# visanalexandru/felics

Hardware: AMD Instinct MI355X
Metric: encode MPix/s on 4K 8-bit grayscale batch (bit-exact); % HBM-read roofline (higher is better)
Workload: dtype u8

## Files before the change

felics_amd/csrc/felics_api.cpp:

```cpp
#include <hip/hip_runtime.h>

#include <chrono>
#include <cstdio>
#include <cstdlib>
#include <cstring>
#include <thread>
#include <type_traits>
#include <string>
#include <algorithm>
#include <new>
#include <tuple>
#include <vector>

#include "../../include/felics.h"
#include "felics_kernels.h"

using namespace felics;

namespace {

enum Stage { ST_PLANES = 0, ST_HIST, ST_OFFSETS, ST_SCATTER, ST_SPINE, ST_ASSIGN, ST_LENGTHS, ST_BITSCAN, ST_ZERO, ST_PACK,
             ST_WIDE_KEYS, ST_WIDE_SORT, ST_WIDE_CHAINS, ST_COUNT };
const char *kStageNames[ST_COUNT] = {"planes", "hist", "offsets", "scatter", "spine", "assign", "lengths", "bitscan", "zero", "pack",
                                     "wide_keys", "wide_sort", "wide_chains"};
static_assert(ST_COUNT <= FELICS_MAX_STAGES, "felics.h promises at most FELICS_MAX_STAGES stages");

constexpr int SLICES = 12;
constexpr uint64_t PASS_MAX_CHAINS = 1u << 23;
constexpr int EV_PAIRS = SLICES + 2;
constexpr int MAX_LANES = 4;
constexpr int DEFAULT_LANES = 2;
int lanes_from_env() {
    if (const char *e = getenv("FELICS_LANES")) return std::max(1, std::min(atoi(e), MAX_LANES));
    return DEFAULT_LANES;
}

struct DevBuf {
    void *p = nullptr;
    size_t cap = 0;
};

struct Lane {
    hipStream_t stream = nullptr;
    hipStream_t front = nullptr;
    hipStream_t kstream = nullptr;
    hipStream_t tail = nullptr;
    hipEvent_t slice_done[SLICES] = {};
    hipEvent_t spine_done[SLICES] = {};
    hipEvent_t assign_done[SLICES] = {};
    hipEvent_t ev[ST_COUNT][EV_PAIRS][2] = {};
    int ev_used[ST_COUNT] = {};
    hipEvent_t sized = nullptr;
    hipEvent_t span_begin = nullptr, span_end = nullptr;
    uint64_t *h_sizes = nullptr;
    size_t h_sizes_cap = 0;
    DevBuf planes, counts, chain_prog, scalars, evs, pix_of, k_map, k_sorted, block_state, group_bits, tile_slots, desc,
        tile_bits, tile_bitoff, plane_sums, image_bytes, image_off, partial, status, edge_first, edge_last, pscratch;
    DevBuf wrecs[2], wtile_cnt, wmeta, whist, wdigtot, heads, wlong;
    uint32_t epoch = 0;
    bool pending = false;
    bool finished = false;
    size_t p_n = 0;
    const void *p_pixels = nullptr;
    uint32_t p_w = 0, p_h = 0;
    int p_color = 0, p_depth = 0;
    uint8_t *p_out = nullptr;
    size_t p_cap = 0;
    uint64_t p_slot = 0;
    std::vector<uint64_t> r_off, r_len;
    int r_rc = 0;
    int nslices = SLICES;
    bool m_tickets = false;
    bool m_fused = false;
    bool queued = false;
    Geometry g;
    size_t first_image = 0;
    const void *d_planes = nullptr;
    DevBuf mtable;
    PlaneGeom *h_table = nullptr;
    size_t h_table_cap = 0;
};

}

struct felics_ctx {
    int device = -1;
    int next_lane = 0;
    int nlanes = DEFAULT_LANES;
    int slices_blocking = 3;
    int slices_queued = 2;
    bool pack_tickets = false;
    bool two_pass = false;
    bool own_tails = false;
    bool serial = false;
    bool test_timeout = false;
    bool test_lookback = false;
    bool scatter_ballot = false;
    bool cap_max = false;
    bool test_tile_cap = false;
    bool test_scatter_order = false;
    bool poison = false;
    bool trace = false;
    int timeout_s = 120;
    bool failed = false;
    felics_stats stats = {};
    Lane lanes[MAX_LANES];
    std::string err;
    bool profiling = false;
    float stage_ms[ST_COUNT] = {};
    float span_ms = 0.f;
    int stage_launches[ST_COUNT] = {};
    DevBuf in, out;
    hipStream_t copy_in = nullptr, copy_out = nullptr;
    std::vector<hipEvent_t> h2d_done;
    hipEvent_t wait_before_submit = nullptr;
    DevBuf mix_in, mix_stage, mix_out, mix_redo;
    DevBuf own;
    DevBuf dec_meta, dec_planes;
    DevBuf dec_planes16;
    DevBuf dec_lane_table;
    DevBuf dec_table;
    uint32_t dec_epoch = 0;
};

namespace {

int hip_fail(felics_ctx *ctx, hipError_t e, const char *what) {
    char buf[256];
    snprintf(buf, sizeof buf, "%s: %s", what, hipGetErrorString(e));
    if (ctx) ctx->err = buf;
    return FELICS_E_HIP;
}

#define HIP_TRY(ctx, call)                                          \
    do {                                                            \
        hipError_t e__ = (call);                                    \
        if (e__ != hipSuccess) return hip_fail(ctx, e__, #call);    \
    } while (0)

int wait_event(felics_ctx *ctx, hipEvent_t ev, const char *what) {
    const auto t0 = std::chrono::steady_clock::now();
    if (ctx->test_timeout) {
        ctx->err = std::string(what) + ": timed out waiting for the GPU; the context is unusable from here on";
        ctx->failed = true;
        ctx->stats.failed = 1;
        return FELICS_E_HIP;
    }
    for (uint32_t spins = 0;; spins++) {
        const hipError_t e = hipEventQuery(ev);
        if (e == hipSuccess) return FELICS_OK;
        if (e != hipErrorNotReady) return hip_fail(ctx, e, what);
        if (spins > 2000) std::this_thread::sleep_for(std::chrono::microseconds(50));
        if ((spins & 1023) == 1023 &&
            std::chrono::steady_clock::now() - t0 > std::chrono::seconds(ctx->timeout_s)) {
            ctx->err = std::string(what) + ": timed out waiting for the GPU; the context is unusable from here on";
            ctx->failed = true;
            ctx->stats.failed = 1;
            return FELICS_E_HIP;
        }
    }
}

int sync_lane(felics_ctx *ctx, Lane &l) {
    if (l.front) HIP_TRY(ctx, hipStreamSynchronize(l.front));
    if (l.stream) HIP_TRY(ctx, hipStreamSynchronize(l.stream));
    if (l.kstream) HIP_TRY(ctx, hipStreamSynchronize(l.kstream));
    if (l.tail) HIP_TRY(ctx, hipStreamSynchronize(l.tail));
    return FELICS_OK;
}

int reserve(felics_ctx *ctx, DevBuf &b, size_t bytes) {
    if (bytes <= b.cap) return FELICS_OK;
    if (b.p) {
        HIP_TRY(ctx, hipFree(b.p));
        b.p = nullptr;
        b.cap = 0;
// ... 7 lines not shown
int reserve_zeroed(felics_ctx *ctx, DevBuf &b, size_t bytes) {
    if (bytes <= b.cap) return FELICS_OK;
    int rc = reserve(ctx, b, bytes);
    if (rc) return rc;
    HIP_TRY(ctx, hipMemset(b.p, 0, b.cap));
    return FELICS_OK;
}

void release(DevBuf &b) {
    if (b.p) (void)hipFree(b.p);
    b.p = nullptr;
    b.cap = 0;
}

struct StageTimer {
    felics_ctx *ctx;
    Lane &lane;
    int st;
    hipStream_t stream;
    int slot = -1;
    bool exact;
    StageTimer(felics_ctx *c, Lane &l, int s, hipStream_t on, bool single_kernel = false)
        : ctx(c), lane(l), st(s), stream(on), exact(single_kernel) {
        if (ctx->profiling && lane.ev_used[st] < EV_PAIRS) {
            slot = lane.ev_used[st]++;
            if (exact)
                g_launch_timing = LaunchTiming{lane.ev[st][slot][0], lane.ev[st][slot][1]};
            else
                (void)hipEventRecord(lane.ev[st][slot][0], stream);
        }
    }
    ~StageTimer() {
        if (slot >= 0) {
            if (!exact) {
                (void)hipEventRecord(lane.ev[st][slot][1], stream);
            } else if (g_launch_timing.start) {
                g_launch_timing = LaunchTiming{};
                lane.ev_used[st]--;
            }
        }
        if (ctx->trace) {
            hipError_t e = hipStreamSynchronize(stream);
            fprintf(stderr, "[felics] %s done (%s)\n", kStageNames[st], hipGetErrorString(e));
        }
    }
};

int check_args(uint32_t w, uint32_t h, int color, int depth) {
    if (color != FELICS_COLOR_GRAY && color != FELICS_COLOR_RGB) return FELICS_E_INVALID_COLOR_TYPE;
    if (depth != FELICS_DEPTH_8 && depth != FELICS_DEPTH_16) return FELICS_E_INVALID_PIXEL_DEPTH;
    if ((uint64_t)w * h > 0xFFFFFFFFull) return FELICS_E_INVALID_DIMENSIONS;
    return FELICS_OK;
}

void header_bytes(uint8_t *o, uint32_t w, uint32_t h, int color, int depth) {
    memcpy(o, "FLCS", 4);
    o[4] = (uint8_t)color;
    o[5] = (uint8_t)depth;
    for (int i = 0; i < 4; i++) {
        o[6 + i] = (uint8_t)(w >> (24 - 8 * i));
        o[10 + i] = (uint8_t)(h >> (24 - 8 * i));
    }
}

template <typename T, typename ET>
int run_lane(felics_ctx *ctx, Lane &l, uint8_t *d_out, uint64_t slot_stride) {
    const Geometry &g = l.g;
    const int ns = l.nslices;
    const size_t nsamples = (size_t)g.nplanes * g.npix;
    int rc = 0;
    const bool fused = (slot_stride != 0 || g.mixed != nullptr) && !ctx->two_pass;
    const uint32_t cap = ctx->cap_max ? tile_cap_max(g.nctx, g.npix) : ctx->test_tile_cap ? std::min(4u * REC, tile_cap_max(g.nctx, g.npix)) : tile_cap_default(g.nctx, g.npix);
    const size_t ptiles = (size_t)g.nplanes * g.sort_tiles;
    const size_t slots = ptiles * cap, recs = slots / REC;
    const size_t nchains = (size_t)g.nplanes * g.nctx;
    if ((rc = reserve(ctx, l.evs, slots * sizeof(ET) + STAGE_PAD)) != 0) return rc;
    if ((rc = reserve(ctx, l.pix_of, slots * 2 + STAGE_PAD)) != 0) return rc;
    if ((rc = reserve(ctx, l.k_sorted, slots + STAGE_PAD)) != 0) return rc;
    if ((rc = reserve(ctx, l.counts, ptiles * g.nctx * 4)) != 0) return rc;
    if ((rc = reserve(ctx, l.tile_slots, ptiles * 4)) != 0) return rc;
    if ((rc = reserve(ctx, l.desc, recs * 8 + 64)) != 0) return rc;
    if ((rc = reserve(ctx, l.block_state, recs * 16 + 64)) != 0) return rc;
    if ((rc = reserve(ctx, l.partial, (size_t)SLICES * nchains * 8)) != 0) return rc;
    if ((rc = reserve(ctx, l.chain_prog, nchains * 32)) != 0) return rc;
    if ((rc = reserve(ctx, l.scalars, 64 + 4 * (SLICES + 2) + 4 * SLICES)) != 0) return rc;
    if (!fused && (rc = reserve(ctx, l.k_map, nsamples + STAGE_PAD)) != 0) return rc;
    if (!fused && (rc = reserve(ctx, l.group_bits, (size_t)g.nplanes * g.pack_tiles * PACK_THREADS * 2)) != 0) return rc;
    if ((rc = reserve(ctx, l.tile_bits, (size_t)g.nplanes * g.pack_tiles * 4)) != 0) return rc;
    if ((rc = reserve(ctx, l.tile_bitoff, (size_t)g.nplanes * g.pack_tiles * 8)) != 0) return rc;
    if ((rc = reserve(ctx, l.plane_sums, (size_t)g.nplanes * 16)) != 0) return rc;
    if ((rc = reserve(ctx, l.image_bytes, (size_t)g.nimages * 8)) != 0) return rc;
    if ((rc = reserve(ctx, l.image_off, (size_t)(g.nimages + 1) * 8)) != 0) return rc;
    if ((rc = reserve_zeroed(ctx, l.status, (size_t)g.nplanes * g.pack_tiles * 8)) != 0) return rc;
    if ((rc = reserve(ctx, l.edge_first, (size_t)g.nplanes * g.pack_tiles * 4)) != 0) return rc;
    if ((rc = reserve(ctx, l.edge_last, (size_t)g.nplanes * g.pack_tiles * 4)) != 0) return rc;
    const size_t hs = (size_t)g.nimages * 2 + 1;
    if (hs > l.h_sizes_cap) {
        if (l.h_sizes) HIP_TRY(ctx, hipHostFree(l.h_sizes));
        l.h_sizes = nullptr;
        HIP_TRY(ctx, hipHostMalloc((void **)&l.h_sizes, hs * 8 + 64, hipHostMallocDefault));
        l.h_sizes_cap = hs;
    }
    hipStream_t s = l.stream, f = l.front, ks = l.kstream, tl = l.tail;
    if (ctx->serial) f = ks = tl = s;
    const T *d_planes = (const T *)l.d_planes;
    auto *chain_state = (uint32_t *)l.chain_prog.p;
    auto *plane_carry = (uint64_t *)l.plane_sums.p;
    auto *plane_base = plane_carry + g.nplanes;
    if (++l.epoch >= 0x03FFFFFFu) l.epoch = 1;
    if ((l.epoch & 0x3FFFFu) == 0) HIP_TRY(ctx, hipMemsetAsync(l.status.p, 0, l.status.cap, f));
    const uint32_t epoch = l.epoch;
    PackTarget target{d_out, slot_stride, nullptr, 0};
    if (fused && g.planes_per_image > 1) {
        target.plane_slot = ((uint64_t)g.npix + g.npix / 4 + 64 + 15) & ~15ull;
        if ((rc = reserve(ctx, l.pscratch, (size_t)(target.plane_slot * g.nimages * (g.planes_per_image - 1)))) != 0) return rc;
        target.scratch = (uint8_t *)l.pscratch.p;
    }
    uint32_t *d_error = (uint32_t *)l.scalars.p + 8;
    uint32_t *d_flags = (uint32_t *)l.scalars.p + 9;
    uint32_t *d_tickets = (uint32_t *)l.scalars.p + 16;
    uint32_t *d_nrec = (uint32_t *)l.scalars.p + 16 + SLICES + 2;
    const TileLocal<ET> tloc{(ET *)l.evs.p, (uint16_t *)l.pix_of.p, (uint8_t *)l.k_sorted.p, (uint32_t *)l.counts.p, (uint32_t *)l.tile_slots.p, cap};
    l.m_tickets = ctx->pack_tickets;
    l.m_fused = fused;

    uint32_t bounds[SLICES + 1];
    for (int q = 0; q <= ns; q++) bounds[q] = (uint32_t)((uint64_t)g.sort_tiles * q / ns);
    auto slice_of = [&](int q) {
        const size_t r0 = (size_t)bounds[q] * g.nplanes * (cap / REC);
        return ChainSlice{(uint2 *)l.desc.p + r0, (uint2 *)l.partial.p + (size_t)q * nchains, d_nrec + q, (uint4 *)l.block_state.p};
    };
    if (ctx->poison) {
        DevBuf *bufs[] = {&l.evs, &l.pix_of, &l.k_sorted, &l.counts, &l.tile_slots, &l.desc, &l.block_state, &l.partial, &l.k_map,
                          &l.group_bits, &l.tile_bits, &l.tile_bitoff, &l.edge_first, &l.edge_last, &l.pscratch};
        for (DevBuf *b : bufs)
            if (b->p) HIP_TRY(ctx, hipMemsetAsync(b->p, 0xA5, b->cap, f));
    }
    HIP_TRY(ctx, hipMemsetAsync(chain_state, 0, nchains * 32, f));
    HIP_TRY(ctx, hipMemsetAsync(d_flags, 0, 4, f));
    HIP_TRY(ctx, hipMemsetAsync(d_nrec, 0, 4 * SLICES, f));
    const uint32_t front_mode = ctx->scatter_ballot ? FRONT_SAFE_RANK : ctx->test_scatter_order ? FRONT_TEST_VIOLATION : 0u;
    if (!ctx->scatter_ballot) ctx->stats.sorted_event_sorts++;
    for (int q = 0; q < ns; q++) {
        if (bounds[q + 1] != bounds[q]) {
            {
                StageTimer t(ctx, l, ST_SCATTER, f, true);
                launch_front<T, ET>(f, d_planes, tloc, g, bounds[q], bounds[q + 1], d_flags, front_mode);
            }
            StageTimer t(ctx, l, ST_OFFSETS, f, true);
            launch_enum(f, tloc.runtab, slice_of(q), g, bounds[q], bounds[q + 1], cap);
        }
        HIP_TRY(ctx, hipEventRecord(l.slice_done[q], f));
    }
    for (int q = 0; q < ns; q++) {
        HIP_TRY(ctx, hipStreamWaitEvent(s, l.slice_done[q], 0));
        if (bounds[q + 1] != bounds[q]) {
            StageTimer t(ctx, l, ST_SPINE, s, true);
            launch_spine3<ET>(s, tloc.ev, slice_of(q), chain_state, d_flags, g);
        }
        HIP_TRY(ctx, hipEventRecord(l.spine_done[q], s));
    }
    for (int q = 0; q < ns; q++) {
        HIP_TRY(ctx, hipStreamWaitEvent(ks, l.spine_done[q], 0));
        if (bounds[q + 1] != bounds[q]) {
            StageTimer t(ctx, l, ST_ASSIGN, ks, true);
            launch_assign3<ET>(ks, tloc, (const uint4 *)l.block_state.p, g, bounds[q], bounds[q + 1]);
        }
        HIP_TRY(ctx, hipEventRecord(l.assign_done[q], ks));
    }
    HIP_TRY(ctx, hipMemsetAsync(plane_carry, 0, (size_t)g.nplanes * 16, tl));
    HIP_TRY(ctx, hipMemsetAsync(d_error, 0, 4, tl));
    HIP_TRY(ctx, hipMemsetAsync(d_tickets, 0, 4 * (SLICES + 2), tl));
    if (fused) {
        for (int q = 0; q < ns; q++) {
            HIP_TRY(ctx, hipStreamWaitEvent(tl, l.assign_done[q], 0));
            if (bounds[q + 1] == bounds[q]) continue;
            StageTimer t(ctx, l, ST_PACK, tl, true);
            launch_pack_t<T>(tl, d_planes, tloc.kq, tloc.pix, tloc.ev, tloc.tile_slots, cap, (uint64_t *)l.status.p, (uint64_t *)l.tile_bitoff.p,
                             (uint32_t *)l.tile_bits.p, plane_carry, (uint32_t *)l.edge_first.p, (uint32_t *)l.edge_last.p, d_error, target, g,
                             bounds[q], bounds[q + 1], epoch, ctx->pack_tickets ? d_tickets + q : nullptr);
        }
        StageTimer t(ctx, l, ST_ZERO, tl);
        launch_finish_sizes(tl, plane_carry, plane_base, (uint64_t *)l.image_bytes.p, g);
        launch_join_edges(tl, (const uint64_t *)l.tile_bitoff.p, (const uint32_t *)l.tile_bits.p,
                          (const uint32_t *)l.edge_first.p, (const uint32_t *)l.edge_last.p, target, g);
        launch_concat_planes(tl, plane_base, plane_carry, target, g);
    } else {
        HIP_TRY(ctx, hipStreamWaitEvent(tl, l.assign_done[ns - 1], 0));
        {
            StageTimer t(ctx, l, ST_ASSIGN, tl, true);
            launch_k_to_pixels_tl(tl, tloc.kq, tloc.pix, tloc.tile_slots, cap, (uint8_t *)l.k_map.p, g);
        }
        {
            StageTimer t(ctx, l, ST_LENGTHS, tl, true);
            launch_lengths<T>(tl, d_planes, (const uint8_t *)l.k_map.p, (uint16_t *)l.group_bits.p,
                              (uint32_t *)l.tile_bits.p, g, 0, g.pack_tiles);
        }
        {
            StageTimer t(ctx, l, ST_BITSCAN, tl);
            launch_bitscan_slice(tl, (const uint32_t *)l.tile_bits.p, (uint64_t *)l.tile_bitoff.p, plane_carry, g, 0, g.pack_tiles);
            launch_finish_sizes(tl, plane_carry, plane_base, (uint64_t *)l.image_bytes.p, g);
        }
        if (slot_stride != 0) {
            {
                StageTimer t(ctx, l, ST_ZERO, tl);
                launch_zero_edges(tl, d_out, nullptr, slot_stride, (const uint64_t *)l.tile_bitoff.p,
                                  (const uint32_t *)l.tile_bits.p, plane_base, g, 0, g.pack_tiles);
            }
            StageTimer t(ctx, l, ST_PACK, tl, true);
            launch_pack<T>(tl, d_planes, (const uint8_t *)l.k_map.p, (const uint16_t *)l.group_bits.p,
                           (const uint64_t *)l.tile_bitoff.p, (const uint32_t *)l.tile_bits.p, plane_base, nullptr,
                           slot_stride, d_out, g, 0, g.pack_tiles);
        }
    }
    HIP_TRY(ctx, hipGetLastError());
    HIP_TRY(ctx, hipMemcpyAsync(l.h_sizes, l.image_bytes.p, (size_t)g.nimages * 8, hipMemcpyDeviceToHost, tl));
    l.h_sizes[g.nimages] = 0;
    HIP_TRY(ctx, hipMemcpyAsync(&l.h_sizes[g.nimages], d_error, 8, hipMemcpyDeviceToHost, tl));
    HIP_TRY(ctx, hipEventRecord(l.sized, tl));
    if (ctx->profiling) HIP_TRY(ctx, hipEventRecord(l.span_end, tl));
    return FELICS_OK;
}

template <typename T>
int run_wide(felics_ctx *ctx, Lane &l, uint8_t *d_out, uint64_t slot_stride) {
    const Geometry &g = l.g;
    const size_t nsamples = (size_t)g.nplanes * g.npix;
    const WideSizes z = wide_sizes(g);
    int rc;
    for (int i = 0; i < 2; i++)
        if ((rc = reserve(ctx, l.wrecs[i], z.rec_bytes)) != 0) return rc;
    if ((rc = reserve(ctx, l.wtile_cnt, z.tile_cnt_bytes)) != 0) return rc;
    if ((rc = reserve(ctx, l.wmeta, z.meta_bytes)) != 0) return rc;
    if ((rc = reserve(ctx, l.whist, z.hist_bytes)) != 0) return rc;
    if ((rc = reserve(ctx, l.wdigtot, z.digtot_bytes)) != 0) return rc;
    if ((rc = reserve(ctx, l.heads, z.heads_bytes)) != 0) return rc;
    if ((rc = reserve(ctx, l.scalars, 64)) != 0) return rc;
    uint32_t lane_limit = wide_lane_limit(g);
    if (const char *e = getenv("FELICS_WIDE_LANE")) lane_limit = (uint32_t)std::max(0, atoi(e));
    const size_t nlong = wide_long_capacity(g, lane_limit);
    if ((rc = reserve(ctx, l.wlong, nlong * (8 + 64) + 64)) != 0) return rc;
    if ((rc = reserve(ctx, l.k_map, nsamples + STAGE_PAD)) != 0) return rc;
    if ((rc = reserve(ctx, l.group_bits, (size_t)g.nplanes * g.pack_tiles * PACK_THREADS * sizeof(group_bits_t<T>))) != 0) return rc;
    if ((rc = reserve(ctx, l.tile_bits, (size_t)g.nplanes * g.pack_tiles * 4)) != 0) return rc;
    if ((rc = reserve(ctx, l.tile_bitoff, (size_t)g.nplanes * g.pack_tiles * 8)) != 0) return rc;
    if ((rc = reserve(ctx, l.plane_sums, (size_t)g.nplanes * 16)) != 0) return rc;
    if ((rc = reserve(ctx, l.image_bytes, (size_t)g.nimages * 8)) != 0) return rc;
    if ((rc = reserve(ctx, l.image_off, (size_t)(g.nimages + 1) * 8)) != 0) return rc;
    const size_t hs = (size_t)g.nimages * 2 + 1;
    if (hs > l.h_sizes_cap) {
        if (l.h_sizes) HIP_TRY(ctx, hipHostFree(l.h_sizes));
        l.h_sizes = nullptr;
        HIP_TRY(ctx, hipHostMalloc((void **)&l.h_sizes, hs * 8 + 64, hipHostMallocDefault));
        l.h_sizes_cap = hs;
    }
    hipStream_t s = l.stream;
    const T *d_planes = (const T *)l.d_planes;
    auto *plane_carry = (uint64_t *)l.plane_sums.p;
    auto *plane_base = plane_carry + g.nplanes;
    auto *nheads = (uint32_t *)l.scalars.p;
    if (ctx->poison) {
        DevBuf *bufs[] = {&l.wrecs[0], &l.wrecs[1], &l.wtile_cnt, &l.wmeta, &l.whist, &l.heads, &l.k_map,
                          &l.group_bits, &l.tile_bits, &l.tile_bitoff};
        for (DevBuf *b : bufs) HIP_TRY(ctx, hipMemsetAsync(b->p, 0xA5, b->cap, s));
    }
    {
        StageTimer t(ctx, l, ST_WIDE_KEYS, s);
        launch_wide_events<T>(s, d_planes, (uint32_t *)l.wtile_cnt.p, (uint32_t *)l.wmeta.p, (uint64_t *)l.wrecs[0].p, g);
    }
    {
        StageTimer t(ctx, l, ST_WIDE_SORT, s);
        launch_wide_sort(s, (uint64_t *)l.wrecs[0].p, (uint64_t *)l.wrecs[1].p, (const uint32_t *)l.wmeta.p, (uint32_t *)l.whist.p,
                         (uint32_t *)l.wdigtot.p, g);
    }
    {
        StageTimer t(ctx, l, ST_WIDE_CHAINS, s);
        HIP_TRY(ctx, hipMemsetAsync(nheads, 0, 8, s));
        launch_wide_chains(s, (const uint64_t *)l.wrecs[0].p, (const uint32_t *)l.wmeta.p, (uint64_t *)l.heads.p, nheads,
                           (uint8_t *)l.k_map.p, g, lane_limit, (uint64_t *)l.wlong.p, (uint32_t *)((uint64_t *)l.wlong.p + nlong));
    }
    HIP_TRY(ctx, hipMemsetAsync(plane_carry, 0, (size_t)g.nplanes * 16, s));
    {
        StageTimer t(ctx, l, ST_LENGTHS, s, true);
        launch_lengths<T>(s, d_planes, (const uint8_t *)l.k_map.p, (group_bits_t<T> *)l.group_bits.p,
                          (uint32_t *)l.tile_bits.p, g, 0, g.pack_tiles);
    }
    {
        StageTimer t(ctx, l, ST_BITSCAN, s);
        launch_bitscan_slice(s, (const uint32_t *)l.tile_bits.p, (uint64_t *)l.tile_bitoff.p, plane_carry, g, 0,
                             g.pack_tiles);
        launch_finish_sizes(s, plane_carry, plane_base, (uint64_t *)l.image_bytes.p, g);
    }
    if (slot_stride != 0) {
        {
            StageTimer t(ctx, l, ST_ZERO, s);
            launch_zero_edges(s, d_out, nullptr, slot_stride, (const uint64_t *)l.tile_bitoff.p,
                              (const uint32_t *)l.tile_bits.p, plane_base, g, 0, g.pack_tiles);
        }
        {
            StageTimer t(ctx, l, ST_PACK, s, true);
            launch_pack<T>(s, d_planes, (const uint8_t *)l.k_map.p, (const group_bits_t<T> *)l.group_bits.p,
                           (const uint64_t *)l.tile_bitoff.p, (const uint32_t *)l.tile_bits.p, plane_base, nullptr,
                           slot_stride, d_out, g, 0, g.pack_tiles);
        }
    }
    HIP_TRY(ctx, hipGetLastError());
    HIP_TRY(ctx, hipMemcpyAsync(l.h_sizes, l.image_bytes.p, (size_t)g.nimages * 8, hipMemcpyDeviceToHost, s));
    HIP_TRY(ctx, hipEventRecord(l.sized, s));
    if (ctx->profiling) HIP_TRY(ctx, hipEventRecord(l.span_end, s));
    return FELICS_OK;
}

template <typename T>
int pack_exact(felics_ctx *ctx, Lane &l, uint8_t *d_out) {
    const Geometry &g = l.g;
    hipStream_t s = l.tail;
    auto *plane_base = (uint64_t *)l.plane_sums.p + g.nplanes;
    {
        StageTimer t(ctx, l, ST_ZERO, s);
        launch_zero_streams(s, (uint32_t *)d_out, (const uint64_t *)l.image_off.p, g);
    }
    {
        StageTimer t(ctx, l, ST_PACK, s, true);
        launch_pack<T>(s, (const T *)l.d_planes, (const uint8_t *)l.k_map.p, (const group_bits_t<T> *)l.group_bits.p,
                       (const uint64_t *)l.tile_bitoff.p, (const uint32_t *)l.tile_bits.p, plane_base,
                       (const uint64_t *)l.image_off.p, 0, d_out, g, 0, g.pack_tiles);
    }
    HIP_TRY(ctx, hipGetLastError());
    return FELICS_OK;
}

void collect_timing(felics_ctx *ctx, Lane &l) {
    if (!ctx->profiling) return;
    ctx->span_ms = 0.f;
    (void)hipEventElapsedTime(&ctx->span_ms, l.span_begin, l.span_end);
    for (int i = 0; i < ST_COUNT; i++) {
        ctx->stage_ms[i] = 0.f;
        ctx->stage_launches[i] = 0;
        for (int k = 0; k < l.ev_used[i]; k++) {
            float ms = 0.f;
            if (hipEventElapsedTime(&ms, l.ev[i][k][0], l.ev[i][k][1]) == hipSuccess) {
                ctx->stage_ms[i] += ms;
                ctx->stage_launches[i]++;
            }
        }
    }
}

size_t max_images_per_pass(uint64_t npix, uint32_t planes, int depth) {
    const uint64_t per_image = npix * planes;
    if (per_image == 0) return SIZE_MAX;
    if (const char *e = getenv("FELICS_TEST_PASS_IMAGES"))
        return (size_t)std::max(1, atoi(e));
    if (depth == FELICS_DEPTH_16) {
        constexpr uint64_t WIDE_MAX_PLANES = 1u << 16;
        return (size_t)std::max<uint64_t>(1, std::min<uint64_t>(0x40000000ull / per_image, WIDE_MAX_PLANES / planes));
    }
    const uint64_t tiles = (npix + SORT_TILE - 1) / SORT_TILE;
    const uint64_t rec_per_image = tiles * planes * (tile_cap_max(NCTX, (uint32_t)std::min<uint64_t>(npix, SORT_TILE)) / REC);
    const uint64_t chains_per_image = (uint64_t)planes * (planes == 3 ? nctx_of<int16_t>() : nctx_of<uint8_t>());
    return (size_t)std::max<uint64_t>(
        1, std::min<uint64_t>({0xE0000000ull / per_image, 0xE0000000ull / rec_per_image, PASS_MAX_CHAINS / chains_per_image}));
}

int launch_sub_batch(felics_ctx *ctx, Lane &l, size_t first, size_t cnt, const void *d_pixels, uint32_t w, uint32_t h,
                     int color, int depth, uint8_t *lane_out, uint64_t slot, int nslices, bool queued = false) {
    l.nslices = std::max(1, std::min(nslices, SLICES));
    l.queued = queued;
    ctx->stats.submissions++;
    const uint32_t planes = color == FELICS_COLOR_RGB ? 3 : 1;
    const uint64_t npix = (uint64_t)w * h;
    const bool wide = depth == FELICS_DEPTH_16;
    const size_t frame_bytes = (size_t)npix * planes * (wide ? 2 : 1);
    int rc;
    Geometry &g = l.g;
    g.mixed = nullptr;
    g.W = w;
    g.H = h;
    g.npix = (uint32_t)npix;
    g.nimages = (uint32_t)cnt;
    g.planes_per_image = planes;
    g.nplanes = (uint32_t)(cnt * planes);
    g.sort_tiles = (uint32_t)((npix + SORT_TILE - 1) / SORT_TILE);
    g.pack_tiles = (uint32_t)((npix + PACK_TILE - 1) / PACK_TILE);
    g.color = (uint32_t)color;
    g.depth = (uint32_t)depth;
    g.nctx = planes == 3 ? nctx_of<int16_t>() : nctx_of<uint8_t>();
    l.first_image = first;
    const uint8_t *src = (const uint8_t *)d_pixels + first * frame_bytes;
    l.d_planes = src;
    if (ctx->wait_before_submit)
        HIP_TRY(ctx, hipStreamWaitEvent(wide || ctx->serial ? l.stream : l.front, ctx->wait_before_submit, 0));
    if (ctx->profiling)
        HIP_TRY(ctx, hipEventRecord(l.span_begin, wide || ctx->serial ? l.stream : l.front));
    if (planes == 3) {
        if ((rc = reserve(ctx, l.planes, (size_t)g.nplanes * npix * (wide ? 4 : 2) + STAGE_PAD)) != 0) return rc;
        hipStream_t fs = wide || ctx->serial ? l.stream : l.front;
        StageTimer t(ctx, l, ST_PLANES, fs, true);
        if (wide)
            launch_rgb16_to_planes(fs, (const uint16_t *)src, (int32_t *)l.planes.p, g.npix, g.nimages);
// ... 817 lines not shown
            for (size_t p = 0; p < rows16.size(); p += per16) {
                const size_t cnt = std::min(per16, rows16.size() - p);
                uint32_t lds = 0, epoch0 = 0;
                uint64_t mx = 0;
                bool rgb = false;
                for (size_t k = p; k < p + cnt; k++) {
                    const size_t i = rows16[k];
                    lds = std::max(lds, decode16_lds_bytes(rec[i].W));
                    mx = std::max(mx, npix[i]);
                    rgb = rgb || rec[i].color;
                }
                int r = dec16_epoch(ctx, w, epoch0);
                if (r) return r;
                HIP_TRY(ctx, launch_decode16_rows(w, st, d_off, d_len, d_rows + rows16_first + p, (uint32_t)cnt, lds, mx, rgb, (uint16_t *)d_pixels,
                                                  (int32_t *)ctx->dec_planes16.p, (uint32_t *)ctx->dec_table.p, epoch0, d_status));
            }
        }
        if (!slots.empty()) {
            hipStream_t w = stream_for();
            HIP_TRY(ctx, hipMemsetAsync(ctx->dec_lane_table.p, 0, lt_bytes, w));
            for (int col = 0; col < 2; col++)
                HIP_TRY(ctx, launch_decode8_lanes_waves(w, st, d_off, d_len, d_waves + lanes[col].first, (uint32_t)lanes[col].cnt, d_slots + slot0[col],
                                                        col, d_rows + conv.first, (uint32_t)conv.cnt, lanes[1].max_npix, d_pixels,
                                                        (int16_t *)ctx->dec_planes.p, (uint32_t *)((uint8_t *)ctx->dec_lane_table.p + (col ? lt_gray : 0)),
                                                        d_status));
        }
        for (const Launch &L : classes)
            HIP_TRY(ctx, launch_decode8_rows(stream_for(), st, d_off, d_len, d_rows + L.first, (uint32_t)L.cnt, L.lds, L.max_npix, L.rgb, d_pixels,
                                             (int16_t *)ctx->dec_planes.p, d_status));
        std::vector<uint8_t> sbuf, pbuf;
        for (size_t i : host) {
            const felics_header want{rec[i].color, rec[i].depth, rec[i].W, rec[i].H};
            const int r = host_decode(ctx, st + offsets[i], lens[i], felics_max_compressed_size(rec[i].W, rec[i].H, rec[i].color, rec[i].depth), want,
                                      d_pixels + pix_offsets[i], sbuf, pbuf);
            if (r == FELICS_E_HIP) return r;
            status[i] = r == HOST_DECODE_NO_MEMORY ? FELICS_E_IO : r;
        }
        const size_t used = std::min(next, work.size());
        for (size_t k = 0; k < used; k++) {
            HIP_TRY(ctx, hipEventRecord(l0.spine_done[k], work[k]));
            HIP_TRY(ctx, hipStreamWaitEvent(s, l0.spine_done[k], 0));
        }
        HIP_TRY(ctx, hipMemcpyAsync(dev_status.data(), d_status, n * 4, hipMemcpyDeviceToHost, s));
        HIP_TRY(ctx, hipStreamSynchronize(s));
        return FELICS_OK;
    };
    if ((rc = queue()) != 0) {
        for (size_t i = 0; i < n; i++) status[i] = FELICS_E_HIP;
        return rc;
    }
    std::vector<char> on_host(n, 0);
    for (size_t i : host) on_host[i] = 1;
    int first = FELICS_OK;
    for (size_t i = 0; i < n; i++) {
        if (!on_host[i]) status[i] = dev_status[i];
        if (status[i] && !first) first = status[i];
    }
    return first;
}

}


extern "C" {

int felics_ctx_create(int device, felics_ctx **out) {
    if (!out) return FELICS_E_INVALID_ARGUMENT;
    *out = nullptr;
    int count = 0;
    hipError_t e = hipGetDeviceCount(&count);
    if (e != hipSuccess || count <= 0 || device < 0 || device >= count) return FELICS_E_HIP;
    felics_ctx *ctx = new (std::nothrow) felics_ctx();
    if (!ctx) return FELICS_E_IO;
    ctx->device = device;
    ctx->nlanes = lanes_from_env();
    ctx->poison = getenv("FELICS_POISON") != nullptr;
    ctx->two_pass = getenv("FELICS_TWO_PASS") != nullptr;
    ctx->test_lookback = getenv("FELICS_TEST_LOOKBACK_FAIL") != nullptr;
    if (const char *e = getenv("FELICS_SCATTER")) ctx->scatter_ballot = !strcmp(e, "ballot");
    ctx->test_tile_cap = getenv("FELICS_TEST_TILE_CAP") != nullptr;
    ctx->test_scatter_order = getenv("FELICS_TEST_SCATTER_ORDER") != nullptr;
    ctx->pack_tickets = ctx->own_tails = getenv("FELICS_OWN_TAILS") != nullptr;
    ctx->serial = getenv("FELICS_SERIAL") != nullptr;
    ctx->test_timeout = getenv("FELICS_TEST_TIMEOUT") != nullptr;
    if (const char *e = getenv("FELICS_SLICES")) ctx->slices_blocking = std::max(1, std::min(atoi(e), SLICES));
    if (const char *e = getenv("FELICS_SLICES_QUEUED")) ctx->slices_queued = std::max(1, std::min(atoi(e), SLICES));
    ctx->trace = getenv("FELICS_TRACE") != nullptr;
    if (const char *e = getenv("FELICS_TIMEOUT_S")) ctx->timeout_s = std::max(1, atoi(e));
    bool ok = hipSetDevice(device) == hipSuccess;
    int prio_low = 0, prio_high = 0;
    (void)hipDeviceGetStreamPriorityRange(&prio_low, &prio_high);
    int prio_spine = prio_high, prio_front = prio_low, prio_tail = prio_high;
    for (int li = 0; li < ctx->nlanes; li++) {
        Lane &l = ctx->lanes[li];
        ok = ok && hipStreamCreateWithPriority(&l.stream, hipStreamNonBlocking, prio_spine) == hipSuccess;
        ok = ok && hipStreamCreateWithPriority(&l.front, hipStreamNonBlocking, prio_front) == hipSuccess;
        ok = ok && hipStreamCreateWithPriority(&l.kstream, hipStreamNonBlocking, prio_tail) == hipSuccess;
        if (&l == &ctx->lanes[0] || ctx->own_tails)
            ok = ok && hipStreamCreateWithPriority(&l.tail, hipStreamNonBlocking, prio_tail) == hipSuccess;
        else
            l.tail = ctx->lanes[0].tail;
        for (int q = 0; q < SLICES && ok; q++) {
            ok = hipEventCreateWithFlags(&l.slice_done[q], hipEventDisableTiming) == hipSuccess;
            ok = ok && hipEventCreateWithFlags(&l.spine_done[q], hipEventDisableTiming) == hipSuccess;
            ok = ok && hipEventCreateWithFlags(&l.assign_done[q], hipEventDisableTiming) == hipSuccess;
        }
        ok = ok && hipEventCreateWithFlags(&l.sized, hipEventDisableTiming) == hipSuccess;
        ok = ok && hipEventCreate(&l.span_begin) == hipSuccess && hipEventCreate(&l.span_end) == hipSuccess;
        for (int i = 0; i < ST_COUNT && ok; i++)
            for (int k = 0; k < EV_PAIRS && ok; k++)
                for (int j = 0; j < 2 && ok; j++) ok = hipEventCreate(&l.ev[i][k][j]) == hipSuccess;
    }
    if (!ok) {
        felics_ctx_destroy(ctx);
        return FELICS_E_HIP;
    }
    *out = ctx;
    return FELICS_OK;
}

void felics_ctx_destroy(felics_ctx *ctx) {
    if (!ctx) return;
    if (ctx->failed) {
        delete ctx;
        return;
    }
    (void)hipSetDevice(ctx->device);
    for (Lane &l : ctx->lanes) {
        if (l.front) (void)hipStreamSynchronize(l.front);
        if (l.stream) (void)hipStreamSynchronize(l.stream);
        if (l.kstream) (void)hipStreamSynchronize(l.kstream);
    }
    for (Lane &l : ctx->lanes)
        if (l.tail) (void)hipStreamSynchronize(l.tail);
    for (Lane &l : ctx->lanes) {
        DevBuf *bufs[] = {&l.planes, &l.counts, &l.chain_prog, &l.scalars, &l.evs, &l.pix_of, &l.k_map, &l.k_sorted, &l.tile_slots, &l.desc,
                          &l.block_state, &l.group_bits, &l.tile_bits, &l.tile_bitoff, &l.plane_sums, &l.image_bytes, &l.image_off,
                          &l.partial, &l.status, &l.edge_first, &l.edge_last, &l.pscratch, &l.wrecs[0], &l.wrecs[1], &l.wtile_cnt, &l.wmeta, &l.whist, &l.wdigtot, &l.heads, &l.wlong};
        for (DevBuf *b : bufs) release(*b);
        if (l.h_sizes) (void)hipHostFree(l.h_sizes);
        release(l.mtable);
        if (l.h_table) (void)hipHostFree(l.h_table);
        for (int i = 0; i < ST_COUNT; i++)
            for (int k = 0; k < EV_PAIRS; k++)
                for (int j = 0; j < 2; j++)
                    if (l.ev[i][k][j]) (void)hipEventDestroy(l.ev[i][k][j]);
        if (l.sized) (void)hipEventDestroy(l.sized);
        if (l.span_begin) (void)hipEventDestroy(l.span_begin);
        if (l.span_end) (void)hipEventDestroy(l.span_end);
        for (int q = 0; q < SLICES; q++) {
            if (l.slice_done[q]) (void)hipEventDestroy(l.slice_done[q]);
            if (l.spine_done[q]) (void)hipEventDestroy(l.spine_done[q]);
            if (l.assign_done[q]) (void)hipEventDestroy(l.assign_done[q]);
        }
        if (l.front) (void)hipStreamDestroy(l.front);
        if (l.kstream) (void)hipStreamDestroy(l.kstream);
        if (l.stream) (void)hipStreamDestroy(l.stream);
        if (l.tail && (&l == &ctx->lanes[0] || l.tail != ctx->lanes[0].tail)) (void)hipStreamDestroy(l.tail);
    }
    release(ctx->in);
    if (ctx->copy_in) (void)hipStreamSynchronize(ctx->copy_in), (void)hipStreamDestroy(ctx->copy_in);
    if (ctx->copy_out) (void)hipStreamSynchronize(ctx->copy_out), (void)hipStreamDestroy(ctx->copy_out);
    for (hipEvent_t ev : ctx->h2d_done)
        if (ev) (void)hipEventDestroy(ev);
    release(ctx->out);
    release(ctx->own);
    release(ctx->mix_in);
    release(ctx->mix_stage);
    release(ctx->mix_out);
    release(ctx->mix_redo);
    release(ctx->dec_meta);
    release(ctx->dec_planes);
    release(ctx->dec_planes16);
    release(ctx->dec_table);
    release(ctx->dec_lane_table);
    delete ctx;
}

size_t felics_max_compressed_size(uint32_t w, uint32_t h, int color, int depth) {
    const uint64_t planes = color == FELICS_COLOR_RGB ? 3 : 1;
    const uint64_t emax = depth == FELICS_DEPTH_8 ? (color ? 509u : 254u) : (color ? 131069u : 65534u);
    const uint64_t px = (uint64_t)w * h;
    const uint64_t bits = planes * 64u + planes * px * (3u + emax);
    return (size_t)(14u + (bits + 7u) / 8u);
}

int felics_compress_batch_device(felics_ctx *ctx, size_t n, const void *d_pixels, uint32_t w, uint32_t h, int color,
                                 int depth, void *d_out, size_t d_out_cap, uint64_t *offsets, uint64_t *lens) {
    if (!ctx || !offsets || !lens || !d_out || (!d_pixels && n && (uint64_t)w * h)) return FELICS_E_INVALID_ARGUMENT;
    if (ctx->failed) return FELICS_E_HIP;
    int rc = check_args(w, h, color, depth);
    if (rc) return rc;
    if (n == 0) return FELICS_OK;
    if (any_pending(ctx)) return FELICS_E_INVALID_ARGUMENT;
    return encode_device(ctx, ctx->lanes[0], n, d_pixels, w, h, color, depth, (uint8_t *)d_out, d_out_cap, offsets, lens,
                         nullptr);
}

int felics_submit_batch_device(felics_ctx *ctx, size_t n, const void *d_pixels, uint32_t w, uint32_t h, int color,
                               int depth, void *d_out, size_t d_out_cap, int *ticket) {
    if (!ctx || !ticket || !d_out || n == 0 || (!d_pixels && (uint64_t)w * h)) return FELICS_E_INVALID_ARGUMENT;
    if (ctx->failed) return FELICS_E_HIP;
    int rc = check_args(w, h, color, depth);
    if (rc) return rc;
    const int L = ctx->next_lane;
    Lane &l = ctx->lanes[L];
    if (l.pending) return FELICS_E_INVALID_ARGUMENT;
    l.p_n = n;
    l.p_pixels = d_pixels;
    l.p_w = w;
    l.p_h = h;
    l.p_color = color;
    l.p_depth = depth;
    l.p_out = (uint8_t *)d_out;
    l.p_cap = d_out_cap;
    l.finished = false;
    const uint32_t planes = color == FELICS_COLOR_RGB ? 3 : 1;
    const uint64_t npix = (uint64_t)w * h;
    const size_t frame_bytes = (size_t)npix * planes * (depth == FELICS_DEPTH_16 ? 2 : 1);
// ... 476 lines not shown
```

Measured before the change: 215,600.

## Coalesce per-run scratch into one cleared block and interleave slice stage issue

Packs image sizes, error/flag words, tickets, plane sums and chain state into a single buffer. This lets one memset clear them all and one device-to-host copy read sizes plus the error word, replacing several small memsets and two copies. Kernel launches are now issued slice by slice (enum, spine, then assign and pack of the previous slice) instead of stage by stage, so downstream streams get work earlier. It also lowers the assign stream's priority and makes its stream selectable. The risk is that changed priorities and issue order could hurt overlap between lanes.

After: 228,500 (median of 6 runs). +6.0%, better.

```diff
diff --git a/felics_amd/csrc/felics_api.cpp b/felics_amd/csrc/felics_api.cpp
--- a/felics_amd/csrc/felics_api.cpp
+++ b/felics_amd/csrc/felics_api.cpp
@@ -30,6 +30,7 @@
 constexpr int EV_PAIRS = SLICES + 2;
 constexpr int MAX_LANES = 4;
 constexpr int DEFAULT_LANES = 2;
+enum AssignOn { ASSIGN_OWN, ASSIGN_FRONT, ASSIGN_TAIL };
 int lanes_from_env() {
     if (const char *e = getenv("FELICS_LANES")) return std::max(1, std::min(atoi(e), MAX_LANES));
     return DEFAULT_LANES;
@@ -54,8 +55,9 @@
     hipEvent_t span_begin = nullptr, span_end = nullptr;
     uint64_t *h_sizes = nullptr;
     size_t h_sizes_cap = 0;
-    DevBuf planes, counts, chain_prog, scalars, evs, pix_of, k_map, k_sorted, block_state, group_bits, tile_slots, desc,
+    DevBuf planes, counts, scalars, evs, pix_of, k_map, k_sorted, block_state, group_bits, tile_slots, desc,
         tile_bits, tile_bitoff, plane_sums, image_bytes, image_off, partial, status, edge_first, edge_last, pscratch;
+    uint64_t *plane_base = nullptr;
     DevBuf wrecs[2], wtile_cnt, wmeta, whist, wdigtot, heads, wlong;
     uint32_t epoch = 0;
     bool pending = false;
@@ -92,6 +94,7 @@
     bool pack_tickets = false;
     bool two_pass = false;
     bool own_tails = false;
+    int assign_on = ASSIGN_OWN;
     bool serial = false;
     bool test_timeout = false;
     bool test_lookback = false;
@@ -265,14 +268,15 @@
     if ((rc = reserve(ctx, l.desc, recs * 8 + 64)) != 0) return rc;
     if ((rc = reserve(ctx, l.block_state, recs * 16 + 64)) != 0) return rc;
     if ((rc = reserve(ctx, l.partial, (size_t)SLICES * nchains * 8)) != 0) return rc;
-    if ((rc = reserve(ctx, l.chain_prog, nchains * 32)) != 0) return rc;
-    if ((rc = reserve(ctx, l.scalars, 64 + 4 * (SLICES + 2) + 4 * SLICES)) != 0) return rc;
     if (!fused && (rc = reserve(ctx, l.k_map, nsamples + STAGE_PAD)) != 0) return rc;
     if (!fused && (rc = reserve(ctx, l.group_bits, (size_t)g.nplanes * g.pack_tiles * PACK_THREADS * 2)) != 0) return rc;
     if ((rc = reserve(ctx, l.tile_bits, (size_t)g.nplanes * g.pack_tiles * 4)) != 0) return rc;
     if ((rc = reserve(ctx, l.tile_bitoff, (size_t)g.nplanes * g.pack_tiles * 8)) != 0) return rc;
-    if ((rc = reserve(ctx, l.plane_sums, (size_t)g.nplanes * 16)) != 0) return rc;
-    if ((rc = reserve(ctx, l.image_bytes, (size_t)g.nimages * 8)) != 0) return rc;
+    const size_t o_words = (size_t)g.nimages * 8, o_counters = o_words + 8;
+    const size_t o_sums = (o_counters + 4 * (2 * SLICES + 2) + 15) & ~(size_t)15;
+    const size_t o_chain = (o_sums + (size_t)g.nplanes * 16 + 255) & ~(size_t)255;
+    const size_t cleared = o_chain + nchains * 32;
+    if ((rc = reserve(ctx, l.image_bytes, cleared)) != 0) return rc;
     if ((rc = reserve(ctx, l.image_off, (size_t)(g.nimages + 1) * 8)) != 0) return rc;
     if ((rc = reserve_zeroed(ctx, l.status, (size_t)g.nplanes * g.pack_tiles * 8)) != 0) return rc;
     if ((rc = reserve(ctx, l.edge_first, (size_t)g.nplanes * g.pack_tiles * 4)) != 0) return rc;
@@ -284,12 +288,15 @@
         HIP_TRY(ctx, hipHostMalloc((void **)&l.h_sizes, hs * 8 + 64, hipHostMallocDefault));
         l.h_sizes_cap = hs;
     }
-    hipStream_t s = l.stream, f = l.front, ks = l.kstream, tl = l.tail;
+    hipStream_t s = l.stream, f = l.front, tl = l.tail;
+    hipStream_t ks = ctx->assign_on == ASSIGN_TAIL ? tl : l.kstream ? l.kstream : f;
     if (ctx->serial) f = ks = tl = s;
     const T *d_planes = (const T *)l.d_planes;
-    auto *chain_state = (uint32_t *)l.chain_prog.p;
-    auto *plane_carry = (uint64_t *)l.plane_sums.p;
+    uint8_t *block = (uint8_t *)l.image_bytes.p;
+    auto *chain_state = (uint32_t *)(block + o_chain);
+    auto *plane_carry = (uint64_t *)(block + o_sums);
     auto *plane_base = plane_carry + g.nplanes;
+    l.plane_base = plane_base;
     if (++l.epoch >= 0x03FFFFFFu) l.epoch = 1;
     if ((l.epoch & 0x3FFFFu) == 0) HIP_TRY(ctx, hipMemsetAsync(l.status.p, 0, l.status.cap, f));
     const uint32_t epoch = l.epoch;
@@ -299,10 +306,10 @@
         if ((rc = reserve(ctx, l.pscratch, (size_t)(target.plane_slot * g.nimages * (g.planes_per_image - 1)))) != 0) return rc;
         target.scratch = (uint8_t *)l.pscratch.p;
     }
-    uint32_t *d_error = (uint32_t *)l.scalars.p + 8;
-    uint32_t *d_flags = (uint32_t *)l.scalars.p + 9;
-    uint32_t *d_tickets = (uint32_t *)l.scalars.p + 16;
-    uint32_t *d_nrec = (uint32_t *)l.scalars.p + 16 + SLICES + 2;
+    uint32_t *d_error = (uint32_t *)(block + o_words);
+    uint32_t *d_flags = d_error + 1;
+    uint32_t *d_tickets = (uint32_t *)(block + o_counters);
+    uint32_t *d_nrec = d_tickets + SLICES + 2;
     const TileLocal<ET> tloc{(ET *)l.evs.p, (uint16_t *)l.pix_of.p, (uint8_t *)l.k_sorted.p, (uint32_t *)l.counts.p, (uint32_t *)l.tile_slots.p, cap};
     l.m_tickets = ctx->pack_tickets;
     l.m_fused = fused;
@@ -319,11 +326,25 @@
         for (DevBuf *b : bufs)
             if (b->p) HIP_TRY(ctx, hipMemsetAsync(b->p, 0xA5, b->cap, f));
     }
-    HIP_TRY(ctx, hipMemsetAsync(chain_state, 0, nchains * 32, f));
-    HIP_TRY(ctx, hipMemsetAsync(d_flags, 0, 4, f));
-    HIP_TRY(ctx, hipMemsetAsync(d_nrec, 0, 4 * SLICES, f));
+    HIP_TRY(ctx, hipMemsetAsync(block, 0, cleared, f));
     const uint32_t front_mode = ctx->scatter_ballot ? FRONT_SAFE_RANK : ctx->test_scatter_order ? FRONT_TEST_VIOLATION : 0u;
     if (!ctx->scatter_ballot) ctx->stats.sorted_event_sorts++;
+    auto behind_spine = [&](int q) -> int {
+        HIP_TRY(ctx, hipStreamWaitEvent(ks, l.spine_done[q], 0));
+        if (bounds[q + 1] != bounds[q]) {
+            StageTimer t(ctx, l, ST_ASSIGN, ks, true);
+            launch_assign3<ET>(ks, tloc, (const uint4 *)l.block_state.p, g, bounds[q], bounds[q + 1]);
+        }
+        HIP_TRY(ctx, hipEventRecord(l.assign_done[q], ks));
+        if (!fused) return FELICS_OK;
+        HIP_TRY(ctx, hipStreamWaitEvent(tl, l.assign_done[q], 0));
+        if (bounds[q + 1] == bounds[q]) return FELICS_OK;
+        StageTimer t(ctx, l, ST_PACK, tl, true);
+        launch_pack_t<T>(tl, d_planes, tloc.kq, tloc.pix, tloc.ev, tloc.tile_slots, cap, (uint64_t *)l.status.p, (uint64_t *)l.tile_bitoff.p,
+                         (uint32_t *)l.tile_bits.p, plane_carry, (uint32_t *)l.edge_first.p, (uint32_t *)l.edge_last.p, d_error, target, g,
+                         bounds[q], bounds[q + 1], epoch, ctx->pack_tickets ? d_tickets + q : nullptr);
+        return FELICS_OK;
+    };
     for (int q = 0; q < ns; q++) {
         if (bounds[q + 1] != bounds[q]) {
             {
@@ -334,35 +355,16 @@
             launch_enum(f, tloc.runtab, slice_of(q), g, bounds[q], bounds[q + 1], cap);
         }
         HIP_TRY(ctx, hipEventRecord(l.slice_done[q], f));
-    }
-    for (int q = 0; q < ns; q++) {
         HIP_TRY(ctx, hipStreamWaitEvent(s, l.slice_done[q], 0));
         if (bounds[q + 1] != bounds[q]) {
             StageTimer t(ctx, l, ST_SPINE, s, true);
             launch_spine3<ET>(s, tloc.ev, slice_of(q), chain_state, d_flags, g);
         }
         HIP_TRY(ctx, hipEventRecord(l.spine_done[q], s));
-    }
-    for (int q = 0; q < ns; q++) {
-        HIP_TRY(ctx, hipStreamWaitEvent(ks, l.spine_done[q], 0));
-        if (bounds[q + 1] != bounds[q]) {
-            StageTimer t(ctx, l, ST_ASSIGN, ks, true);
-            launch_assign3<ET>(ks, tloc, (const uint4 *)l.block_state.p, g, bounds[q], bounds[q + 1]);
-        }
-        HIP_TRY(ctx, hipEventRecord(l.assign_done[q], ks));
-    }
-    HIP_TRY(ctx, hipMemsetAsync(plane_carry, 0, (size_t)g.nplanes * 16, tl));
-    HIP_TRY(ctx, hipMemsetAsync(d_error, 0, 4, tl));
-    HIP_TRY(ctx, hipMemsetAsync(d_tickets, 0, 4 * (SLICES + 2), tl));
+        if (q > 0 && (rc = behind_spine(q - 1)) != 0) return rc;
+    }
+    if ((rc = behind_spine(ns - 1)) != 0) return rc;
     if (fused) {
-        for (int q = 0; q < ns; q++) {
-            HIP_TRY(ctx, hipStreamWaitEvent(tl, l.assign_done[q], 0));
-            if (bounds[q + 1] == bounds[q]) continue;
-            StageTimer t(ctx, l, ST_PACK, tl, true);
-            launch_pack_t<T>(tl, d_planes, tloc.kq, tloc.pix, tloc.ev, tloc.tile_slots, cap, (uint64_t *)l.status.p, (uint64_t *)l.tile_bitoff.p,
-                             (uint32_t *)l.tile_bits.p, plane_carry, (uint32_t *)l.edge_first.p, (uint32_t *)l.edge_last.p, d_error, target, g,
-                             bounds[q], bounds[q + 1], epoch, ctx->pack_tickets ? d_tickets + q : nullptr);
-        }
         StageTimer t(ctx, l, ST_ZERO, tl);
         launch_finish_sizes(tl, plane_carry, plane_base, (uint64_t *)l.image_bytes.p, g);
         launch_join_edges(tl, (const uint64_t *)l.tile_bitoff.p, (const uint32_t *)l.tile_bits.p,
@@ -397,9 +399,8 @@
         }
     }
     HIP_TRY(ctx, hipGetLastError());
-    HIP_TRY(ctx, hipMemcpyAsync(l.h_sizes, l.image_bytes.p, (size_t)g.nimages * 8, hipMemcpyDeviceToHost, tl));
     l.h_sizes[g.nimages] = 0;
-    HIP_TRY(ctx, hipMemcpyAsync(&l.h_sizes[g.nimages], d_error, 8, hipMemcpyDeviceToHost, tl));
+    HIP_TRY(ctx, hipMemcpyAsync(l.h_sizes, block, o_counters, hipMemcpyDeviceToHost, tl));
     HIP_TRY(ctx, hipEventRecord(l.sized, tl));
     if (ctx->profiling) HIP_TRY(ctx, hipEventRecord(l.span_end, tl));
     return FELICS_OK;
@@ -441,6 +442,7 @@
     const T *d_planes = (const T *)l.d_planes;
     auto *plane_carry = (uint64_t *)l.plane_sums.p;
     auto *plane_base = plane_carry + g.nplanes;
+    l.plane_base = plane_base;
     auto *nheads = (uint32_t *)l.scalars.p;
     if (ctx->poison) {
         DevBuf *bufs[] = {&l.wrecs[0], &l.wrecs[1], &l.wtile_cnt, &l.wmeta, &l.whist, &l.heads, &l.k_map,
@@ -498,7 +500,7 @@
 int pack_exact(felics_ctx *ctx, Lane &l, uint8_t *d_out) {
     const Geometry &g = l.g;
     hipStream_t s = l.tail;
-    auto *plane_base = (uint64_t *)l.plane_sums.p + g.nplanes;
+    const uint64_t *plane_base = l.plane_base;
     {
         StageTimer t(ctx, l, ST_ZERO, s);
         launch_zero_streams(s, (uint32_t *)d_out, (const uint64_t *)l.image_off.p, g);
@@ -1482,6 +1484,8 @@
     ctx->test_scatter_order = getenv("FELICS_TEST_SCATTER_ORDER") != nullptr;
     ctx->pack_tickets = ctx->own_tails = getenv("FELICS_OWN_TAILS") != nullptr;
     ctx->serial = getenv("FELICS_SERIAL") != nullptr;
+    ctx->assign_on = ctx->nlanes > 3 ? ASSIGN_FRONT : ASSIGN_OWN;
+    if (const char *e = getenv("FELICS_ASSIGN_STREAM")) ctx->assign_on = !strcmp(e, "tail") ? ASSIGN_TAIL : !strcmp(e, "front") ? ASSIGN_FRONT : ASSIGN_OWN;
     ctx->test_timeout = getenv("FELICS_TEST_TIMEOUT") != nullptr;
     if (const char *e = getenv("FELICS_SLICES")) ctx->slices_blocking = std::max(1, std::min(atoi(e), SLICES));
     if (const char *e = getenv("FELICS_SLICES_QUEUED")) ctx->slices_queued = std::max(1, std::min(atoi(e), SLICES));
@@ -1490,12 +1494,13 @@
     bool ok = hipSetDevice(device) == hipSuccess;
     int prio_low = 0, prio_high = 0;
     (void)hipDeviceGetStreamPriorityRange(&prio_low, &prio_high);
-    int prio_spine = prio_high, prio_front = prio_low, prio_tail = prio_high;
+    int prio_spine = prio_high, prio_front = prio_low, prio_tail = ctx->nlanes > 3 && !ctx->own_tails ? (prio_low + prio_high) / 2 : prio_high;
+    const int prio_assign = prio_low;
     for (int li = 0; li < ctx->nlanes; li++) {
         Lane &l = ctx->lanes[li];
         ok = ok && hipStreamCreateWithPriority(&l.stream, hipStreamNonBlocking, prio_spine) == hipSuccess;
         ok = ok && hipStreamCreateWithPriority(&l.front, hipStreamNonBlocking, prio_front) == hipSuccess;
-        ok = ok && hipStreamCreateWithPriority(&l.kstream, hipStreamNonBlocking, prio_tail) == hipSuccess;
+        if (ctx->assign_on == ASSIGN_OWN) ok = ok && hipStreamCreateWithPriority(&l.kstream, hipStreamNonBlocking, prio_assign) == hipSuccess;
         if (&l == &ctx->lanes[0] || ctx->own_tails)
             ok = ok && hipStreamCreateWithPriority(&l.tail, hipStreamNonBlocking, prio_tail) == hipSuccess;
         else
@@ -1534,7 +1539,7 @@
     for (Lane &l : ctx->lanes)
         if (l.tail) (void)hipStreamSynchronize(l.tail);
     for (Lane &l : ctx->lanes) {
-        DevBuf *bufs[] = {&l.planes, &l.counts, &l.chain_prog, &l.scalars, &l.evs, &l.pix_of, &l.k_map, &l.k_sorted, &l.tile_slots, &l.desc,
+        DevBuf *bufs[] = {&l.planes, &l.counts, &l.scalars, &l.evs, &l.pix_of, &l.k_map, &l.k_sorted, &l.tile_slots, &l.desc,
                           &l.block_state, &l.group_bits, &l.tile_bits, &l.tile_bitoff, &l.plane_sums, &l.image_bytes, &l.image_off,
                           &l.partial, &l.status, &l.edge_first, &l.edge_last, &l.pscratch, &l.wrecs[0], &l.wrecs[1], &l.wtile_cnt, &l.wmeta, &l.whist, &l.wdigtot, &l.heads, &l.wlong};
         for (DevBuf *b : bufs) release(*b);
```
